# Reefufui/image_denoising_filter

Hardware: AMD Instinct MI355X
Metric: Mpixel/s (NLM 21x21 search / 7x7 patch, 1920x1080 RGBA32F) (higher is better)
Workload: dtype f32

## Files before the change

### image_denoising_filter_amd/csrc/nlm_strip.hpp

```cpp
#pragma once
#include "common.hpp"
#include "nlm_vbox_plan.hpp"
#include <cmath>
#include <cstdlib>
#include <type_traits>
#include <utility>

namespace mid {

constexpr int kFmtRuntime = -1;
constexpr int kNlmWalk = 21;

struct NlmArgs {
    int w, h;
    float kexp;
    float sk, inv_sk;
    int tiles_x, tiles_y;
    unsigned wg_first;
    const void *target;
    const void *neighbour;
    mid_weightinfo *W;
    int slo, shi;
    int n_frames, k, first, count;
    int out_fmt;
    int corunning;
    int fmt;
    FrameTable frames;
    OutTable outs;
};

template <int PW, int R>
__device__ __forceinline__ void vertical_box(const float (&D)[R + PW - 1], float (&V)[R])
{
    constexpr int N = R + PW - 1;
    float S[N], Pf[N];
#pragma unroll
    for (int m = N - 1; m >= 0; --m) {
        const bool block_end = (m % PW == PW - 1) || (m == N - 1);
        S[m] = block_end ? D[m] : D[m] + S[m + 1];
    }
#pragma unroll
    for (int m = 0; m < N; ++m) {
        const bool block_start = (m % PW == 0);
        Pf[m] = block_start ? D[m] : Pf[m - 1] + D[m];
    }
#pragma unroll
    for (int k = 0; k < R; ++k) {
        if (k % PW == 0) V[k] = (k == 0) ? S[0] : Pf[k + PW - 1];
        else V[k] = S[k] + Pf[k + PW - 1];
    }
}

template <class F, int... I>
__device__ __forceinline__ void static_for_impl(F &&f, std::integer_sequence<int, I...>) { (f(std::integral_constant<int, I>{}), ...); }
template <int N, class F>
__device__ __forceinline__ void static_for(F &&f) { static_for_impl(f, std::make_integer_sequence<int, N>{}); }

template <int PLO, int PHI>
__device__ __forceinline__ float horizontal_box(float v)
{
    constexpr int NL = -PLO, NR = PHI - 1;
    float c = v;
#pragma unroll
    for (int i = 0; i < NR; ++i) c = v + wave_shl1(c);
    if constexpr (NL > 0) {
        float b = v;
#pragma unroll
        for (int i = 0; i < NL - 1; ++i) b = v + wave_shr1(b);
        c = c + wave_shr1(b);
    }
    return c;
}

constexpr int nlm_min_waves(bool rts, bool multi, int pw)
{
    return (rts && multi && (pw == 4 || pw == 5 || pw >= 7)) ? 2 : 1;
}

template <int SLO, int SHI, int PLO, int PHI, int R, int NW, int FMT, bool FUSED, bool MULTI, bool HALF = false, int TAG = 0>
__global__ __launch_bounds__(NW * 64) __attribute__((amdgpu_waves_per_eu(nlm_min_waves(SLO == 0 && SHI == 0, MULTI, PHI - PLO), 2)))
void nlm_strip_kernel(const NlmArgs a)
{
    constexpr bool RTS = (SLO == 0 && SHI == 0);
    constexpr int PW = PHI - PLO;
    constexpr int DR = R + PW - 1;
    constexpr int NL = -PLO, NR = PHI - 1;
    constexpr int VW = 64 - (PW - 1);
    constexpr int TILE_H = NW * R;
    const int slo = RTS ? a.slo : SLO;
    const int SW = RTS ? a.shi - a.slo : SHI - SLO;
    const int LW = 64 + SW - 1;
    const int LH = TILE_H + PW - 1 + SW - 1;
    static_assert(PLO <= 0 && PHI >= 1 && (RTS || SHI - SLO >= 1), "ranges must contain 0");
    static_assert(!HALF || (R == 4 && NW == 8), "HALF: eight waves of four rows");
    static_assert(FMT != kFmtRuntime || RTS, "only the run-time-window instantiations take the format as an argument");

    extern __shared__ float4 lds[];

    const int tid = threadIdx.x, lane = tid & 63, wv = tid >> 6;
    const unsigned tiles = (unsigned)(a.tiles_x * a.tiles_y);
    const unsigned bid = blockIdx.x + a.wg_first;
    const int fz = (int)(bid / tiles);
    const unsigned trem = xcd_remap_in_frame(bid - (unsigned)fz * tiles, tiles, (unsigned)fz);
    const int ty = (int)(trem / (unsigned)a.tiles_x), tx = (int)(trem - (unsigned)ty * a.tiles_x);

    const int w = a.w, h = a.h;
    const int X0 = tx * VW, Y0 = ty * TILE_H;
    const int gx = X0 + PLO + lane;
    const int yb = Y0 + wv * R;
    const bool wave_active = yb < h;

    const int t_out = a.first + fz;
    const void *target = FUSED ? a.frames.p[t_out] : a.target;
    int f_lo = FUSED ? t_out : 0, f_hi = f_lo;
    if (FUSED && MULTI) {
        f_lo = t_out - a.k < 0 ? 0 : t_out - a.k;
        f_hi = t_out + a.k > a.n_frames - 1 ? a.n_frames - 1 : t_out + a.k;
    }

    float Tr[DR], Tg[DR], Tb[DR];
    if constexpr (FMT == kFmtRuntime) {
        if (a.fmt == MID_FMT_RGBA8) {
#pragma unroll
            for (int m = 0; m < DR; ++m) {
                const float4 t = fetch_texture<MID_FMT_RGBA8>(target, w, h, gx, yb + PLO + m);
                Tr[m] = t.x * a.sk; Tg[m] = t.y * a.sk; Tb[m] = t.z * a.sk;
            }
        } else if (a.fmt == MID_FMT_RGBA16F) {
#pragma unroll
            for (int m = 0; m < DR; ++m) {
                const float4 t = fetch_texture<MID_FMT_RGBA16F>(target, w, h, gx, yb + PLO + m);
                Tr[m] = t.x * a.sk; Tg[m] = t.y * a.sk; Tb[m] = t.z * a.sk;
            }
        } else {
#pragma unroll
            for (int m = 0; m < DR; ++m) {
                const float4 t = fetch_texture<MID_FMT_RGBA32F>(target, w, h, gx, yb + PLO + m);
                Tr[m] = t.x * a.sk; Tg[m] = t.y * a.sk; Tb[m] = t.z * a.sk;
            }
        }
    } else {
#pragma unroll
        for (int m = 0; m < DR; ++m) {
            const float4 t = fetch_texture<FMT>(target, w, h, gx, yb + PLO + m);
            Tr[m] = t.x * a.sk; Tg[m] = t.y * a.sk; Tb[m] = t.z * a.sk;
        }
    }
    auto fill = [&](const void *nb, bool *opaque) {
        if constexpr (FMT == kFmtRuntime) {
            if (a.fmt == MID_FMT_RGBA8) fill_tile<MID_FMT_RGBA8, false>(lds, LW, LH, nb, w, h, X0 + PLO + slo, Y0 + PLO + slo, tid, NW * 64, a.sk, opaque);
            else if (a.fmt == MID_FMT_RGBA16F) fill_tile<MID_FMT_RGBA16F, false>(lds, LW, LH, nb, w, h, X0 + PLO + slo, Y0 + PLO + slo, tid, NW * 64, a.sk, opaque);
            else fill_tile<MID_FMT_RGBA32F, false>(lds, LW, LH, nb, w, h, X0 + PLO + slo, Y0 + PLO + slo, tid, NW * 64, a.sk, opaque);
        } else {
            fill_tile<FMT, false>(lds, LW, LH, nb, w, h, X0 + PLO + slo, Y0 + PLO + slo, tid, NW * 64, a.sk, opaque);
        }
    };

    float4 tot[R];
    float totw[R];
#pragma unroll
    for (int k = 0; k < R; ++k) { tot[k] = make_float4(0.f, 0.f, 0.f, 0.f); totw[k] = 0.f; }

    for (int f = f_lo; f <= f_hi; ++f) {
        const void *nb = FUSED ? a.frames.p[f] : a.neighbour;
        __syncthreads();
        constexpr bool kOpaqueForm = !RTS;
        bool opaque = false;
        if constexpr (kOpaqueForm) {
            bool mine = true;
            fill(nb, &mine);
            opaque = __syncthreads_and(mine) != 0;
        } else {
            fill(nb, nullptr);
            __syncthreads();
        }
        if (!wave_active) continue;

        float4 acc[R];
        float accw[R];
#pragma unroll
        for (int k = 0; k < R; ++k) { acc[k] = make_float4(0.f, 0.f, 0.f, 0.f); accw[k] = 0.001f; }

        auto raise_priority = [] { __builtin_amdgcn_sched_barrier(0); __builtin_amdgcn_s_setprio(1); __builtin_amdgcn_sched_barrier(0); };
        auto drop_priority = [] { __builtin_amdgcn_sched_barrier(0); __builtin_amdgcn_s_setprio(0); __builtin_amdgcn_sched_barrier(0); };

        constexpr int WALK = (!RTS && SHI - SLO < kNlmWalk) ? SHI - SLO : kNlmWalk;
        constexpr bool EARLY = NL >= 1;
        const bool lower_half = HALF && (__builtin_amdgcn_readfirstlane(wv) & 1) != 0;
        auto step = [&](auto LT, auto A1, int j, float4 (&n)[DR], const float4 *nextp, bool more) {
            constexpr int OFF = (HALF && decltype(LT)::value) ? 4 : 0;
            using Plan = VboxPlanOf<PW, HALF ? 8 : R, OFF, OFF + R>;
            constexpr int N = Plan::plan.n;
            constexpr bool FOLD = Plan::plan.folded > 0;
            float S[N], Pf[N], D[N];
            auto add_row = [&](auto I) {
                constexpr int i = decltype(I)::value, m = Plan::order.row[i];
                constexpr VboxRow row = Plan::plan.row[m];
                if constexpr (Plan::order.is_s[i]) {
                    if constexpr (row.s_from < 0) S[m] = D[m]; else S[m] = D[m] + S[row.s_from];
                } else {
                    if constexpr (row.p_from < 0) Pf[m] = D[m]; else Pf[m] = Pf[row.p_from] + D[m];
                }
            };
            static_for<Plan::order.count>([&](auto I) {
                constexpr int i = decltype(I)::value, m = Plan::order.row[i];
                constexpr VboxRow row = Plan::plan.row[m];
                const float4 &t = n[(j + m - OFF) % DR];
                if constexpr (row.single) {
                    const float dx = Tr[m - OFF] - t.x, dy = Tg[m - OFF] - t.y, dz = Tb[m - OFF] - t.z;
                    if constexpr (Plan::order.is_s[i]) S[m] = fmaf(dz, dz, fmaf(dy, dy, fmaf(dx, dx, S[row.s_from])));
                    else Pf[m] = fmaf(dz, dz, fmaf(dy, dy, fmaf(dx, dx, Pf[row.p_from])));
                } else {
                    if constexpr (Plan::order.first[i]) {
                        const float dx = Tr[m - OFF] - t.x, dy = Tg[m - OFF] - t.y, dz = Tb[m - OFF] - t.z;
                        D[m] = fmaf(dz, dz, fmaf(dy, dy, dx * dx));
                    }
                    if constexpr (FOLD) add_row(I);
                }
            });
            if constexpr (EARLY) {
                asm volatile("" ::"v"(n[j % DR].w));
                if (more) n[j % DR] = nextp[0];
            }
            if constexpr (!FOLD) raise_priority();
            if constexpr (!FOLD) static_for<Plan::order.count>(add_row);
            float V[R];
            static_for<R>([&](auto K) {
                constexpr int k = decltype(K)::value + OFF;
                if constexpr (Plan::plan.v_uses_s(k) && Plan::plan.v_uses_p(k)) V[k - OFF] = S[k] + Pf[k + PW - 1];
                else if constexpr (Plan::plan.v_uses_s(k)) V[k - OFF] = S[k];
                else V[k - OFF] = Pf[k + PW - 1];
            });
            if constexpr (FOLD) raise_priority();
            float dd[R], ww[R];
#pragma unroll
            for (int k = 0; k < R; ++k) dd[k] = horizontal_box<PLO, PHI>(V[k]);
#pragma unroll
            for (int k = 0; k < R; ++k) ww[k] = __builtin_amdgcn_exp2f(-dd[k]);
#pragma unroll
            for (int k = 0; k < R; ++k) {
                const float wt = ww[k];
                const float4 c = n[(j + k + NL) % DR];
                acc[k].x = fmaf(c.x, wt, acc[k].x); acc[k].y = fmaf(c.y, wt, acc[k].y);
                acc[k].z = fmaf(c.z, wt, acc[k].z); acc[k].w = fmaf(c.w, wt, acc[k].w);
                if constexpr (!decltype(A1)::value) accw[k] += wt;
            }
            if constexpr (!EARLY) { if (more) n[j % DR] = nextp[0]; }
            drop_priority();
        };
        auto run = [&](auto LT, auto A1, const bool FULL, const float4 *colp, int steps) __attribute__((always_inline)) {
            float4 n[DR];
#pragma unroll
            for (int m = 0; m < DR; ++m) n[m] = colp[m * LW];
#pragma unroll
            for (int j = 0; j < WALK; ++j) {
                if (FULL || j < steps) step(LT, A1, j, n, colp + (DR + j) * LW, FULL ? j + 1 < WALK : j + 1 < steps);
            }
            const float last_w = decltype(A1)::value ? acc[R - 1].w : accw[R - 1];
#pragma unroll
            for (int m = 0; m < DR; ++m) asm volatile("" ::"v"(n[m].w), "v"(last_w));
        };
        auto walk = [&](auto A1) {
            for (int sy0 = 0; sy0 < SW; sy0 += WALK) {
                const int steps = sy0 + WALK < SW ? WALK : SW - sy0;
                const float4 *rowp = lds + (wv * R + sy0) * LW + lane;
                if (HALF && lower_half) {
                    if (steps == WALK) { for (int sx = 0; sx < SW; ++sx) run(std::bool_constant<HALF>{}, A1, true, rowp + sx, steps); }
                    else { for (int sx = 0; sx < SW; ++sx) run(std::bool_constant<HALF>{}, A1, false, rowp + sx, steps); }
                } else {
                    if (steps == WALK) { for (int sx = 0; sx < SW; ++sx) run(std::false_type{}, A1, true, rowp + sx, steps); }
                    else { for (int sx = 0; sx < SW; ++sx) run(std::false_type{}, A1, false, rowp + sx, steps); }
                }
            }
        };
        if (kOpaqueForm && opaque) {
            walk(std::true_type{});
#pragma unroll
            for (int k = 0; k < R; ++k) accw[k] = 0.001f + acc[k].w;
        } else {
            walk(std::false_type{});
        }
#pragma unroll
        for (int k = 0; k < R; ++k) {
            acc[k].x *= a.inv_sk; acc[k].y *= a.inv_sk; acc[k].z *= a.inv_sk;
            if (MULTI) {
                tot[k].x += acc[k].x; tot[k].y += acc[k].y; tot[k].z += acc[k].z; tot[k].w += acc[k].w;
                totw[k] += accw[k];
            } else {
                tot[k] = acc[k];
                totw[k] = accw[k];
            }
        }
        if (!MULTI) break;
    }

    if (wave_active && lane >= NL && lane <= 63 - NR && gx < w) {
#pragma unroll
        for (int k = 0; k < R; ++k) {
            const int gy = yb + k;
            if (gy >= h) break;
            const size_t idx = (size_t)gy * w + gx;
            if (FUSED) {
                float4 o;
                if (totw[k] == 0.0f) o = make_float4(1.f, 0.f, 1.f, 1.f);
                else o = make_float4(tot[k].x / totw[k], tot[k].y / totw[k], tot[k].z / totw[k], tot[k].w / totw[k]);
                if (a.out_fmt == MID_FMT_RGBA8) ((uint32_t *)a.outs.p[fz])[idx] = pack_rgba8(o);
                else if (a.out_fmt == MID_FMT_RGBA16F) ((uint2 *)a.outs.p[fz])[idx] = pack_rgba16f(o);
                else ((float4 *)a.outs.p[fz])[idx] = o;
            } else {
                float4 *wp = (float4 *)(a.W + idx);
                float4 wc = wp[0], nw = wp[1];
                wc.x += tot[k].x; wc.y += tot[k].y; wc.z += tot[k].z; wc.w += tot[k].w;
                nw.x += totw[k];
                wp[0] = wc;
                wp[1] = nw;
            }
        }
    }
}

template <int SLO, int SHI, int PLO, int PHI, int R, int NW, int FMT, bool FUSED, bool MULTI, bool HALF = false, int TAG = 0>
static int launch_strip(mid_ctx *ctx, NlmArgs &a, hipStream_t s, unsigned wg_first = 0, unsigned wg_count = ~0u)
{
    constexpr bool RTS = (SLO == 0 && SHI == 0);
    constexpr int PW = PHI - PLO;
    constexpr int VW = 64 - (PW - 1), TILE_H = NW * R;
    const int SW = RTS ? a.shi - a.slo : SHI - SLO;
    const int LW = 64 + SW - 1, LH = TILE_H + PW - 1 + SW - 1;
    const size_t lds_bytes = (size_t)LW * LH * sizeof(float4);
    auto kern = nlm_strip_kernel<SLO, SHI, PLO, PHI, R, NW, FMT, FUSED, MULTI, HALF, TAG>;
    if ((int)lds_bytes > ctx->lds_max)
        return set_error(MID_ERR_UNSUPPORTED, "nlm tile needs %zu B of LDS, device offers %d", lds_bytes, ctx->lds_max);
    if (int rc = ensure_lds(ctx, (const void *)kern, RTS ? (size_t)ctx->lds_max : lds_bytes)) return rc;
    a.tiles_x = (int)cdiv(a.w, VW);
    a.tiles_y = (int)cdiv(a.h, TILE_H);
    const unsigned nwg = (unsigned)a.tiles_x * a.tiles_y * (FUSED ? a.count : 1);
    if (wg_first >= nwg) return MID_OK;
    const unsigned n = wg_count < nwg - wg_first ? wg_count : nwg - wg_first;
    if (n == 0) return MID_OK;
    a.wg_first = wg_first;
    hipLaunchKernelGGL(kern, dim3(n), dim3(NW * 64), lds_bytes, s, a);
    a.wg_first = 0;
    MID_HIP(hipGetLastError());
    return MID_OK;
}

inline unsigned nlm_tile_workgroups(int w, int h, int patch_w, int frames)
{
    return cdiv((unsigned)w, (unsigned)(64 - (patch_w - 1))) * cdiv((unsigned)h, 32u) * (unsigned)frames;
}

int nlm_dispatch_rt8(mid_ctx *ctx, const mid_nlm_params *p, NlmArgs &a, hipStream_t s, bool fused, bool *handled);
int nlm_dispatch_rt4(mid_ctx *ctx, const mid_nlm_params *p, NlmArgs &a, hipStream_t s, bool fused, bool *handled);
constexpr unsigned kNlmSmallRounds = 7;
int nlm_dispatch_small(mid_ctx *ctx, const mid_nlm_params *p, NlmArgs &a, hipStream_t s, int fmt, bool fused, bool *handled);

}
```

Measured before the change: 4973.

## Pack two mostly-empty right-edge tiles into one NLM workgroup

When the last tile column holds at most 16 useful columns, two vertically adjacent edge tiles are packed into one workgroup. Lanes are split into 16-wide groups, each with its own LDS sub-tile fill and output ownership. This cuts the number of launched workgroups that would mostly compute padding. It adds index arithmetic and branching for all workgroups, plus a special fill path.

```diff
diff --git a/image_denoising_filter_amd/csrc/nlm_strip.hpp b/image_denoising_filter_amd/csrc/nlm_strip.hpp
--- a/image_denoising_filter_amd/csrc/nlm_strip.hpp
+++ b/image_denoising_filter_amd/csrc/nlm_strip.hpp
@@ -25,6 +25,7 @@
     int out_fmt;
     int corunning;
     int fmt;
+    int edge;
     FrameTable frames;
     OutTable outs;
 };
@@ -70,6 +71,40 @@
         c = c + wave_shr1(b);
     }
     return c;
+}
+
+constexpr int kNlmEdgeB = 48;
+constexpr bool nlm_edge_packs(int w, int tiles_x, int vw, int pw, int sw)
+{
+    return w - (tiles_x - 1) * vw + (pw - 1) <= 16 && 2 * (16 + sw - 1) <= 64 + sw - 1;
+}
+constexpr unsigned nlm_frame_workgroups(int tiles_x, int tiles_y, bool edge)
+{
+    return edge ? (unsigned)((tiles_x - 1) * tiles_y + (tiles_y + 1) / 2) : (unsigned)(tiles_x * tiles_y);
+}
+
+template <int FMT>
+__device__ __forceinline__ void fill_edge_pair(float4 *lds, int tw, int th, int sub_w, const void *img, int w, int h,
+                                               int x0, int y0a, int y0b, int tid, int nthreads, float rgb_scale)
+{
+    const int n = tw * th, half = kNlmEdgeB;
+    for (int t0 = tid; t0 < n; t0 += 4 * nthreads) {
+        float4 v[4];
+#pragma unroll
+        for (int j = 0; j < 4; ++j) {
+            const int t = t0 + j * nthreads;
+            const int ty = t / tw, tx = t - ty * tw;
+            const bool second = tx >= half;
+            const int c = second ? tx - half : tx;
+            v[j] = make_float4(0.f, 0.f, 0.f, 0.f);
+            if (t < n && c < sub_w) v[j] = fetch_texture<FMT>(img, w, h, x0 + c, (second ? y0b : y0a) + ty);
+        }
+#pragma unroll
+        for (int j = 0; j < 4; ++j) {
+            const int t = t0 + j * nthreads;
+            if (t < n) lds[t] = make_float4(v[j].x * rgb_scale, v[j].y * rgb_scale, v[j].z * rgb_scale, v[j].w);
+        }
+    }
 }
 
 constexpr int nlm_min_waves(bool rts, bool multi, int pw)
@@ -97,18 +132,29 @@
 
     extern __shared__ float4 lds[];
 
+    constexpr bool kEdge = !HALF && TAG == 0;
+    const bool packed = kEdge && a.edge != 0;
+
     const int tid = threadIdx.x, lane = tid & 63, wv = tid >> 6;
-    const unsigned tiles = (unsigned)(a.tiles_x * a.tiles_y);
+    const unsigned tiles = packed ? nlm_frame_workgroups(a.tiles_x, a.tiles_y, true) : (unsigned)(a.tiles_x * a.tiles_y);
     const unsigned bid = blockIdx.x + a.wg_first;
     const int fz = (int)(bid / tiles);
     const unsigned trem = xcd_remap_in_frame(bid - (unsigned)fz * tiles, tiles, (unsigned)fz);
-    const int ty = (int)(trem / (unsigned)a.tiles_x), tx = (int)(trem - (unsigned)ty * a.tiles_x);
+    const unsigned cols = (unsigned)a.tiles_x - (packed ? 1u : 0u);
+    const unsigned blk = packed ? trem / (2u * cols + 1u) : 0u, inblk = trem - blk * (2u * cols + 1u);
+    const unsigned blk_rows = (unsigned)a.tiles_y - 2u * blk < 2u ? 1u : 2u;
+    const bool edge_wg = packed && inblk == blk_rows * cols;
+    const int ty = packed ? 2 * (int)blk + (edge_wg ? 0 : (int)(inblk / cols)) : (int)(trem / cols);
+    const int tx = edge_wg ? a.tiles_x - 1 : packed ? (int)(inblk - (unsigned)(ty - 2 * (int)blk) * cols) : (int)(trem - (unsigned)ty * cols);
 
     const int w = a.w, h = a.h;
     const int X0 = tx * VW, Y0 = ty * TILE_H;
-    const int gx = X0 + PLO + lane;
-    const int yb = Y0 + wv * R;
-    const bool wave_active = yb < h;
+    const int sub = lane & 15, grp = (lane >> 4) & 1;
+    const int gx = X0 + PLO + (edge_wg ? sub : lane);
+    const int yb = Y0 + (edge_wg ? grp * TILE_H : 0) + wv * R;
+    const int lcol = lane - (edge_wg ? (lane & 48) - grp * kNlmEdgeB : 0);
+    const bool owner = edge_wg ? (lane < 32 && sub >= NL && sub <= 15 - NR) : (lane >= NL && lane <= 63 - NR);
+    const bool wave_active = Y0 + wv * R < h;
 
     const int t_out = a.first + fz;
     const void *target = FUSED ? a.frames.p[t_out] : a.target;
@@ -147,6 +193,18 @@
         }
     }
     auto fill = [&](const void *nb, bool *opaque) {
+        if (kEdge && edge_wg) {
+            if (opaque) *opaque = false;
+            const int sub_w = 16 + SW - 1, x0 = X0 + PLO + slo, y0 = Y0 + PLO + slo;
+            if constexpr (FMT == kFmtRuntime) {
+                if (a.fmt == MID_FMT_RGBA8) fill_edge_pair<MID_FMT_RGBA8>(lds, LW, LH, sub_w, nb, w, h, x0, y0, y0 + TILE_H, tid, NW * 64, a.sk);
+                else if (a.fmt == MID_FMT_RGBA16F) fill_edge_pair<MID_FMT_RGBA16F>(lds, LW, LH, sub_w, nb, w, h, x0, y0, y0 + TILE_H, tid, NW * 64, a.sk);
+                else fill_edge_pair<MID_FMT_RGBA32F>(lds, LW, LH, sub_w, nb, w, h, x0, y0, y0 + TILE_H, tid, NW * 64, a.sk);
+            } else {
+                fill_edge_pair<FMT>(lds, LW, LH, sub_w, nb, w, h, x0, y0, y0 + TILE_H, tid, NW * 64, a.sk);
+            }
+            return;
+        }
         if constexpr (FMT == kFmtRuntime) {
             if (a.fmt == MID_FMT_RGBA8) fill_tile<MID_FMT_RGBA8, false>(lds, LW, LH, nb, w, h, X0 + PLO + slo, Y0 + PLO + slo, tid, NW * 64, a.sk, opaque);
             else if (a.fmt == MID_FMT_RGBA16F) fill_tile<MID_FMT_RGBA16F, false>(lds, LW, LH, nb, w, h, X0 + PLO + slo, Y0 + PLO + slo, tid, NW * 64, a.sk, opaque);
@@ -263,7 +321,7 @@
         auto walk = [&](auto A1) {
             for (int sy0 = 0; sy0 < SW; sy0 += WALK) {
                 const int steps = sy0 + WALK < SW ? WALK : SW - sy0;
-                const float4 *rowp = lds + (wv * R + sy0) * LW + lane;
+                const float4 *rowp = lds + (wv * R + sy0) * LW + lcol;
                 if (HALF && lower_half) {
                     if (steps == WALK) { for (int sx = 0; sx < SW; ++sx) run(std::bool_constant<HALF>{}, A1, true, rowp + sx, steps); }
                     else { for (int sx = 0; sx < SW; ++sx) run(std::bool_constant<HALF>{}, A1, false, rowp + sx, steps); }
@@ -294,7 +352,7 @@
         if (!MULTI) break;
     }
 
-    if (wave_active && lane >= NL && lane <= 63 - NR && gx < w) {
+    if (wave_active && owner && gx < w) {
 #pragma unroll
         for (int k = 0; k < R; ++k) {
             const int gy = yb + k;
@@ -334,7 +392,8 @@
     if (int rc = ensure_lds(ctx, (const void *)kern, RTS ? (size_t)ctx->lds_max : lds_bytes)) return rc;
     a.tiles_x = (int)cdiv(a.w, VW);
     a.tiles_y = (int)cdiv(a.h, TILE_H);
-    const unsigned nwg = (unsigned)a.tiles_x * a.tiles_y * (FUSED ? a.count : 1);
+    a.edge = !HALF && TAG == 0 && nlm_edge_packs(a.w, a.tiles_x, VW, PW, SW);
+    const unsigned nwg = nlm_frame_workgroups(a.tiles_x, a.tiles_y, a.edge != 0) * (FUSED ? a.count : 1);
     if (wg_first >= nwg) return MID_OK;
     const unsigned n = wg_count < nwg - wg_first ? wg_count : nwg - wg_first;
     if (n == 0) return MID_OK;
```

After: 4985, median of 6. Within noise of the previous version (+0.2%).
